# zlib-ng/minizip-ng

Measured on NVIDIA H100. Metric: deflate_l1_crc32_input_throughput, higher is better.
Workload: dtype u8

## Files before the change

### minizip-ng_b200/csrc/deflate_kernel.cuh

```cuda
#ifndef MZ_DEFLATE_KERNEL_CUH
#define MZ_DEFLATE_KERNEL_CUH

#include "mzcuda_common.cuh"

namespace mzc {

constexpr int DF_THREADS = 512;
constexpr int DF_WARPS = DF_THREADS / 32;
constexpr int DF_CHUNK_MAX = 65536;
constexpr int DF_UNIT = 32768;
constexpr int DF_SB = DF_UNIT;
constexpr int DF_SPAN = 8;
constexpr int DF_BATCH = DF_THREADS * DF_SPAN;
constexpr int DF_NBATCH = DF_UNIT / DF_BATCH;
constexpr int DF_MINMATCH = 4;
constexpr int DF_LOCKLEN = 8;
constexpr int DF_HASH_BITS = 13;
constexpr int DF_HASH_ENTRIES = 1 << DF_HASH_BITS;
constexpr int DF_STAGE_WORDS = DF_UNIT / 4 + 64;
constexpr int DF_HDR_WORDS = 96;

constexpr uint32_t DF_FLAG_FINAL = 1u;
constexpr uint32_t DF_FLAG_DICT = 2u;

constexpr int DF_OFF_IN = 0;
constexpr int DF_OFF_HASH = DF_OFF_IN + DF_UNIT + 64;
constexpr int DF_OFF_STAGE = DF_OFF_HASH;
constexpr int DF_OFF_REC = DF_OFF_HASH + DF_STAGE_WORDS * 4;
constexpr int DF_OFF_SPN = DF_OFF_REC + DF_NBATCH * DF_THREADS * 8;
constexpr int DF_SPAN_BYTES = DF_NBATCH * DF_THREADS * 10;
constexpr int DF_OFF_HIST = DF_OFF_REC + DF_SPAN_BYTES;
constexpr int DF_OFF_HIST2 = DF_OFF_HIST + (288 + 32) * 4;
constexpr int DF_OFF_CODE = DF_OFF_HIST2 + 256 * 4;
constexpr int DF_OFF_LENS = DF_OFF_CODE + (288 + 32) * 4;
constexpr int DF_OFF_BITS = DF_OFF_LENS + (288 + 32);
constexpr int DF_OFF_SCAN = DF_OFF_BITS + (288 + 32);
constexpr int DF_OFF_BB = DF_OFF_SCAN + 256 * 4;
constexpr int DF_OFF_MISC = DF_OFF_BB + 512 * 4;
constexpr int DF_OFF_SINK = DF_OFF_MISC + 32 * 4 + 16;
constexpr int DF_OFF_LSYM = DF_OFF_SINK + 32 * 4;
constexpr int DF_SMEM_BYTES = DF_OFF_LSYM + 256 * 2;
constexpr int DF_OFF_CAPL = DF_OFF_HIST;
static_assert(DF_OFF_CAPL + DF_WARPS * DF_NBATCH * 32 <= DF_OFF_SCAN, "capped-span lists fit in front of the scan scratch");
constexpr uint32_t DF_ZERO_SYM = 286;
static_assert(DF_HASH_ENTRIES * 4 <= DF_STAGE_WORDS * 4, "hash fits the staging region");
constexpr int DFH_PREV = 32768;
constexpr int DFH_HASH_BITS = 14;
constexpr int DFH_OFF_HASH = (DF_SMEM_BYTES + 15) & ~15;
constexpr int DFH_SMEM_BYTES = DFH_PREV + DFH_OFF_HASH + (4 << DFH_HASH_BITS);
static_assert(DFH_SMEM_BYTES <= 227 * 1024, "shared memory budget of the history variant");
static_assert(DF_SMEM_BYTES <= 113 * 1024, "shared memory budget for two CTAs per SM");

enum { MISC_CHUNK = 3, MISC_CARRY = 8  };

struct DeflateParams {
    const uint8_t *in;
    const uint64_t *in_off;
    const uint32_t *in_len;
    const uint8_t *flags;
    uint64_t total_len;
    uint32_t chunk_size;
    uint32_t nchunks;
    uint32_t last_flags;
    int32_t level;
    uint8_t *out;
    uint64_t slot_stride;
    uint32_t *out_len;
    uint32_t *work_counter;
};

__host__ __device__ inline uint64_t deflate_slot_bound(uint32_t chunk_size) {
    return (((uint64_t)chunk_size + 12ull * ((chunk_size + DF_SB - 1) / DF_SB + 1) + 64 + 15) & ~15ull);
}

__device__ __forceinline__ void length_symbol(uint32_t len, uint32_t &sym, uint32_t &ebits, uint32_t &eval) {
    const uint32_t l = len - 3;
    const uint32_t msb = 31u - (uint32_t)__clz((int)(l | 4u));
    uint32_t e = msb - 2;
    uint32_t sy = 4 * (e + 1) + ((l >> e) & 3u);
    uint32_t ev = l & ((1u << e) - 1u);
    sy = l < 8 ? l : sy;
    const bool top = len == 258;
    sym = top ? 28u : sy;
    ebits = top ? 0u : e;
    eval = top ? 0u : ev;
}
__device__ __forceinline__ void dist_symbol0(uint32_t d, uint32_t &sym, uint32_t &ebits) {
    uint32_t m = 31u - (uint32_t)__clz((int)(d | 1u));
    ebits = m > 0 ? m - 1 : 0u;
    sym = 2 * m + ((d >> ebits) & 1u);
}
__device__ __forceinline__ uint32_t len_extra_bits(uint32_t lsym) { return (lsym < 8 || lsym >= 28) ? 0u : (lsym >> 2) - 1; }
__device__ __forceinline__ uint32_t dist_extra_bits(uint32_t dsym) { return dsym < 4 ? 0u : (dsym >> 1) - 1; }

__device__ __forceinline__ uint32_t stage_word(uint32_t base, uint32_t pos, uint32_t k4) { return base + __umulhi(pos, 1u << 27) * k4; }

__device__ __forceinline__ void stage_put(uint32_t *stage, uint32_t pos, uint32_t v, uint32_t n) {
    if (n == 0) return;
    if (n < 32) v &= (1u << n) - 1;
    uint32_t w = pos >> 5, s = pos & 31;
    atomicOr(&stage[w], v << s);
    if (s + n > 32) atomicOr(&stage[w + 1], v >> (32 - s));
}

__device__ __forceinline__ void stage_or(const Smem &sm, uint32_t pos, uint32_t v, uint32_t n) {
    const uint32_t sh = pos & 31u, wa = DF_OFF_STAGE + ((pos >> 5) << 2);
    sm.red_or32(wa, v << sh);
    if (sh + n > 32) sm.red_or32(wa + 4, v >> (32 - sh));
}

struct BitWriter {
    Smem sm;
    uint64_t acc;
    uint32_t nb, wa;
    __device__ __forceinline__ void init(const Smem &s, uint32_t bitoff) {
        sm = s; wa = DF_OFF_STAGE + (bitoff >> 5) * 4; nb = bitoff & 31; acc = 0;
    }
    __device__ __forceinline__ void put(uint32_t v, uint32_t n) {
        acc |= (uint64_t)v << nb;
        nb += n;
        if (nb >= 32) {
            sm.red_or32(wa, (uint32_t)acc);
            acc >>= 32; nb -= 32; wa += 4;
        }
    }
    __device__ __forceinline__ uint32_t bitpos() const { return ((wa - (uint32_t)DF_OFF_STAGE) << 3) + nb; }
    __device__ __forceinline__ void finish() {
        if (nb > 0) sm.red_or32(wa, (uint32_t)acc);
        if (nb > 32) sm.red_or32(wa + 4, (uint32_t)(acc >> 32));
    }
};

enum { DF_PH_LOAD, DF_PH_PARSE, DF_PH_M0, DF_PH_COVER, DF_PH_T_M1, DF_PH_D, DF_PH_EMIT, DF_PH_FLUSH, DF_PH_UNITS,
       DF_PH_D_STATS, DF_PH_D_SWEEP1, DF_PH_D_SWEEP2, DF_PH_D_KRAFT, DF_PH_D_CANON, DF_PH_D_PASSES,
       DF_PH_P_A = DF_PH_D_PASSES + 8, DF_PH_P_B, DF_PH_P_C, DF_PH_M_INDEX, DF_PH_M_NEAR, DF_PH_M_EXTEND, DF_PH_X_SCAN, DF_PH_X_EMIT,
       DF_PH_X_M3, DF_PH_COLS };
constexpr int DF_PH_ROWS = 1024;
#if defined(MZ_DF_PHASES) && !defined(MZ_EMU)
__device__ unsigned long long g_df_phases[DF_PH_ROWS][DF_PH_COLS];
#define DF_PHASE_BEGIN(t) unsigned long long t = clock64()
#define DF_PHASE(t, ph)                                                                        \
    do {                                                                                       \
        if (threadIdx.x == 0 && blockIdx.x < (unsigned)DF_PH_ROWS) {                           \
            const unsigned long long now_ = clock64();                                         \
            atomicAdd(&g_df_phases[blockIdx.x][ph], now_ - (t));                               \
            if ((ph) == DF_PH_LOAD) atomicAdd(&g_df_phases[blockIdx.x][DF_PH_UNITS], 1ull);   \
            (t) = now_;                                                                        \
        }                                                                                      \
    } while (0)
#define DF_PHASE_COUNT(col)                                                                                          \
    do {                                                                                                             \
        if (threadIdx.x == 0 && blockIdx.x < (unsigned)DF_PH_ROWS) atomicAdd(&g_df_phases[blockIdx.x][col], 1ull); \
    } while (0)
#else
#define DF_PHASE_BEGIN(t)
#define DF_PHASE(t, ph)
#define DF_PHASE_COUNT(col)
#endif

constexpr int DF_BB_THREADS = 320;
enum { BB_STAT = 0 , BB_KRAFT = 8 , BB_SLACK = 136 ,
       BB_CNTW = 144 ,
       BB_NZ = 464 , BB_ST = 474 ,
       BB_HSUM = 484 , BB_HDRBITS = 494 ,
       BB_TOKBITS = 495 , BB_TOKW = 496  };

constexpr uint64_t CL_LENS = 0x12ddad91b725bb4ull;
constexpr uint64_t CL_CODE_LO = 0x840013930ef3c6ull, CL_CODE_HI = 0xd5c7fdf6cb149ull;
constexpr uint64_t CL_ORDER57 = 0x1b6d6db248db92dull;
__device__ __forceinline__ uint32_t cl_len(uint32_t s) { return (uint32_t)(CL_LENS >> (3 * s)) & 7u; }
__device__ __forceinline__ uint32_t cl_code(uint32_t s) {
    return s < 10 ? (uint32_t)(CL_CODE_LO >> (6 * s)) & 63u : (uint32_t)(CL_CODE_HI >> (6 * (s - 10))) & 63u;
}

__device__ __forceinline__ void bb_count_lengths(uint32_t *cntw_row, uint32_t L, unsigned lane, unsigned &m) {
    if (lane < 16) cntw_row[lane] = 0;
    __syncwarp();
    m = __match_any_sync(MZ_FULL_MASK, L);
    if (L > 0 && lane == (unsigned)(__ffs((int)m) - 1)) cntw_row[L] = (uint32_t)__popc(m);
    __syncwarp();
}

__device__ inline void block_build_codes(const uint32_t *hist_ll, const uint32_t *hist_lit2, const uint32_t *hist_d, uint8_t *lens_ll, uint8_t *lens_d,
                                         uint32_t *code_ll, uint32_t *code_d, uint8_t *bits_ll, uint8_t *bits_d, uint32_t *bb,
                                         uint32_t *stage, uint32_t hdrpos, uint32_t bfinal) {
    const uint32_t tid = threadIdx.x;
    const unsigned lane = lane_id(), w = warp_id();
    const int a = tid < 288 ? 0 : (tid < 320 ? 1 : 2);
    const uint32_t sym = a == 0 ? tid : tid - 288;
    const uint32_t nsym = a == 0 ? 286u : 30u;
    const int M = 15;
    const uint32_t one = 1u << M;
    const uint32_t w0 = a == 0 ? 0u : 9u;
    uint32_t c = (a < 2 && sym < nsym) ? (a == 0 ? hist_ll[sym] + (sym < 256 ? hist_lit2[sym] : 0u) : hist_d[sym]) : 0u;
    DF_PHASE_BEGIN(d_t);

    if (tid < 144) bb[tid] = (tid == BB_STAT + 2 || tid == BB_STAT + 6) ? 0xffffffffu : 0u;
    bar_sync(1, DF_BB_THREADS);
    if (a < 2) {
        uint32_t used_w = __reduce_add_sync(MZ_FULL_MASK, c ? 1u : 0u);
        uint32_t tot_w = __reduce_add_sync(MZ_FULL_MASK, c);
        uint32_t first_w = __reduce_min_sync(MZ_FULL_MASK, c ? sym : 0xffffffffu);
        if (lane == 0) {
            atomicAdd(&bb[BB_STAT + a * 4 + 0], used_w);
            atomicAdd(&bb[BB_STAT + a * 4 + 1], tot_w);
            atomicMin(&bb[BB_STAT + a * 4 + 2], first_w);
        }
    }
    bar_sync(1, DF_BB_THREADS);
    DF_PHASE(d_t, DF_PH_D_STATS);
    float ideal = 0.f;
    if (a < 2) {
        uint32_t used = bb[BB_STAT + a * 4 + 0], total = bb[BB_STAT + a * 4 + 1], fu = bb[BB_STAT + a * 4 + 2];
        if (used < 2) {
            uint32_t d0 = used == 0 ? 0u : (fu == 0 ? 1u : 0u);
            uint32_t d1 = used == 0 ? 1u : d0;
            if ((sym == d0 || sym == d1) && c == 0) c = 1;
            total += 2 - used;
        }
// ... 217 lines not shown
        len += 4;
    }
    return len < maxlen ? len : maxlen;
}

__device__ __forceinline__ uint32_t sel_u32(bool p, uint32_t a, uint32_t b) {
#ifdef MZ_EMU
    return p ? a : b;
#else
    uint32_t r;
    asm("{\n.reg .pred q;\nsetp.ne.u32 q, %3, 0;\nselp.b32 %0, %1, %2, q;\n}" : "=r"(r) : "r"(a), "r"(b), "r"((uint32_t)p));
    return r;
#endif
}

__device__ __forceinline__ uint32_t opaque4() { return blockDim.x / (uint32_t)(DF_THREADS / 4); }

template <bool HIST>
__device__ __forceinline__ uint32_t hash_addr(uint32_t v, uint32_t k4) {
    return (HIST ? DFH_OFF_HASH : DF_OFF_HASH) + __umulhi(v * 2654435761u, 1u << (HIST ? DFH_HASH_BITS : DF_HASH_BITS)) * k4;
}

__device__ __forceinline__ uint32_t rec_len(uint32_t r) { uint32_t l = (r >> 3) & 255u; return l ? l + 3 : 0u; }

__device__ __forceinline__ uint32_t fin_len(uint32_t m) { return ((m >> 4) & 255u) + 3u; }
__device__ __forceinline__ uint32_t fin_dist(uint32_t m) { return ((m >> 12) & 0x7fffu) + 1u; }
template <bool ONEM>
__device__ __forceinline__ void span_classify(const Smem &sm, uint32_t A, uint32_t B, uint32_t q0, uint32_t cover, uint32_t &F, uint32_t &MA,
                                              uint32_t &MB) {
    const uint32_t lit = (A >> 26) | ((B >> 26) << 6);
    const uint32_t crel = cover > q0 ? cover - q0 : 0u;
    const uint32_t cr8 = crel < 8 ? crel : 8u;
    uint32_t ex = 0;
    MA = MB = 0;
#pragma unroll
    for (int r = 0; r < (ONEM ? 1 : 2); r++) {
        const uint32_t R = r == 0 ? A : B;
        const uint32_t j = R & 7u, end = j + rec_len(R);
        const uint32_t s = j > crel ? j : crel;
        const uint32_t Lf = (end > s ? end : s) - s;
        const uint32_t P = (s < 8u ? s : 8u) & 7u;
        const uint32_t M = Lf >= 3 ? (((Lf << 4) + (0x80000000u - (3u << 4))) | P | ((R << 1) & (0x7fffu << 12))) : 0u;
        if (r == 0) MA = M;
        else MB = M;
        ex = Lf - 1u < 2u ? Lf : ex;
    }
    F = ((lit >> cr8) << cr8) | (ex << 8);
    if (ex) {
        const uint32_t p = DF_OFF_IN + q0 + crel;
        F |= sm.ld8(p) << 16;
        if (ex == 2) F |= sm.ld8(p + 1) << 24;
    }
}

__device__ __forceinline__ uint32_t match_symbols(const Smem &sm, uint32_t M) {
    uint32_t ds, db;
    const uint32_t lsv = sm.ld16(DF_OFF_LSYM + ((M >> 3) & 0x1feu));
    const uint32_t d = fin_dist(M) - 1;
    dist_symbol0(d, ds, db);
    sm.red_add32(DF_OFF_HIST + (257u + (lsv & 31u)) * 4, 1u);
    sm.red_add32(DF_OFF_HIST + (288u + ds) * 4, 1u);
    return 0x80000000u | ((M & 7u) << 28) | ((d & ((1u << db) - 1u)) << 15) | (ds << 10) | lsv;
}
__device__ __forceinline__ uint32_t match_bits(const Smem &sm, uint32_t M) {
    const uint32_t n = sm.ld8(DF_OFF_BITS + 257u + (M & 31u)) + sm.ld8(DF_OFF_BITS + 288u + ((M >> 10) & 31u));
    return M ? n : 0u;
}
__device__ __forceinline__ void put_match_bits(const Smem &sm, uint32_t pos, uint32_t M) {
    const uint32_t cwl = sm.ld32(DF_OFF_CODE + (257u + (M & 31u)) * 4);
    const uint32_t cwd = sm.ld32(DF_OFF_CODE + (288u + ((M >> 10) & 31u)) * 4);
    const uint32_t cl = (cwl >> 16) & 15u, cd = (cwd >> 16) & 15u;
    const uint32_t v1 = (cwl & 0x7fffu) | (((M >> 5) & 31u) << cl);
    const uint32_t n1 = cl + ((cwl >> 20) & 15u);
    const uint32_t v2 = (cwd & 0x7fffu) | (((M >> 15) & 0x1fffu) << cd);
    const uint64_t V = (uint64_t)v1 | ((uint64_t)v2 << n1);
    const uint32_t lo = (uint32_t)V, hi = (uint32_t)(V >> 32);
    const uint32_t wa = stage_word(DF_OFF_STAGE, pos, opaque4());
    const uint32_t w0 = __funnelshift_l(0u, lo, pos), w1 = __funnelshift_l(lo, hi, pos), w2 = __funnelshift_l(hi, 0u, pos);
    sm.red_or32(wa, w0);
    sm.red_or32(wa + 4, w1);
    if (w2) sm.red_or32(wa + 8, w2);
}

__device__ __forceinline__ uint32_t nth_parked(const uint32_t (&bm)[DF_NBATCH], uint32_t k, uint32_t warp) {
    uint32_t r = k, word = 0, bsel = 0;
    bool found = false;
#pragma unroll
    for (int b = 0; b < DF_NBATCH; b++) {
        const uint32_t c = (uint32_t)__popc(bm[b]);
        const bool here = !found && r < c;
        word = here ? bm[b] : word;
        bsel = here ? (uint32_t)b : bsel;
        found = found || here;
        r -= found ? 0u : c;
    }
    uint32_t base = 0;
#pragma unroll
    for (int st = 16; st; st >>= 1) {
        const uint32_t c = (uint32_t)__popc((word >> base) & ((1u << st) - 1u));
        const bool up = r >= c;
        r -= up ? c : 0u;
        base += up ? (uint32_t)st : 0u;
    }
    return found ? bsel * (uint32_t)DF_THREADS + warp * 32u + base : 0xffffffffu;
}

struct SpanBits {
    uint32_t v[4], E0, E1, offs, xv, MA, size;
};
template <bool ONEM>
__device__ __forceinline__ SpanBits span_bits(const Smem &sm, uint32_t sidx, uint32_t F, uint32_t MA, uint32_t MB, uint32_t code_base, uint32_t zero_ent,
                                              uint32_t k4) {
    SpanBits s;
    const uint2 x = sm.ld64(DF_OFF_IN + sidx * DF_SPAN);
    uint32_t xn = 0;
    s.xv = 0;
    const uint32_t ex = (F >> 8) & 3u;
    if (ex) {
        const uint32_t c0 = sm.ld32(DF_OFF_CODE + ((F >> 16) & 0xffu) * 4);
        s.xv = c0 & 0x7fffu;
        xn = (c0 >> 16) & 15u;
        if (ex == 2) {
            const uint32_t c1 = sm.ld32(DF_OFF_CODE + (F >> 24) * 4);
            s.xv |= (c1 & 0x7fffu) << xn;
            xn += (c1 >> 16) & 15u;
        }
    }
    uint32_t cw[8];
#pragma unroll
    for (int j = 0; j < 8; j++) {
        const uint32_t by = MZ_BYTE(j < 4 ? x.x : x.y, j & 3);
        cw[j] = sm.ld32_a(((F >> j) & 1u) ? by * k4 + code_base : zero_ent);
    }
    const uint32_t nA = match_bits(sm, MA), nB = ONEM ? 0u : match_bits(sm, MB);
    const uint32_t sA = MA ? ((MA >> 28) & 7u) * 8u : 64u, sB = MB ? ((MB >> 28) & 7u) * 8u : 64u;
    const uint32_t L0 = __byte_perm(__byte_perm(cw[0], cw[1], 0x0062u), __byte_perm(cw[2], cw[3], 0x0062u), 0x5410u) + shl_clamp(nA, sA) + shl_clamp(nB, sB);
    const uint32_t L1 = __byte_perm(__byte_perm(cw[4], cw[5], 0x0062u), __byte_perm(cw[6], cw[7], 0x0062u), 0x5410u) + shl_clamp(nA, sA - 32u) + shl_clamp(nB, sB - 32u);
    const uint32_t P0 = L0 * 0x01010101u;
    const uint32_t P1 = L1 * 0x01010101u + (P0 >> 24) * 0x01010101u;
    s.E0 = P0 << 8;
    s.E1 = __funnelshift_l(P0, P1, 8);
#pragma unroll
    for (int jj = 0; jj < 4; jj++) {
        const uint32_t c0 = cw[2 * jj], c1 = cw[2 * jj + 1];
        s.v[jj] = (c0 & 0xffffu) | ((c1 & 0xffffu) << (c0 >> 16));
    }
    s.offs = xn + (((shr_clamp(s.E0, sA) & 0xffu) + (shr_clamp(s.E1, sA - 32u) & 0xffu)) << 8) +
             (((shr_clamp(s.E0, sB) & 0xffu) + (shr_clamp(s.E1, sB - 32u) & 0xffu)) << 16);
    s.MA = MA;
    s.size = xn + (P1 >> 24);
    return s;
}
template <bool ONEM>
__device__ __forceinline__ void span_emit(const Smem &sm, const SpanBits &s, uint32_t pos, uint32_t sidx, uint32_t stage_base, uint32_t k4) {
    const uint32_t xn = s.offs & 0xffu;
    if (xn) stage_or(sm, pos, s.xv, xn);
    pos += xn;
#pragma unroll
    for (int jj = 0; jj < 4; jj++) {
        const uint32_t pp = pos + MZ_BYTE(jj < 2 ? s.E0 : s.E1, 2 * (jj & 1));
        const uint32_t wa = stage_word(stage_base, pp, k4);
        sm.red_or32_a(wa, __funnelshift_l(0u, s.v[jj], pp));
        sm.red_or32_a(wa + 4, __funnelshift_l(s.v[jj], 0u, pp));
    }
    if (s.MA) put_match_bits(sm, pos + ((s.offs >> 8) & 0xffu), s.MA);
    if (!ONEM) sm.st32(DF_OFF_REC + sidx * 8, pos + (s.offs >> 16));
}

template <int STRIDE, bool LAZY, bool HIST = false>
__global__ void __launch_bounds__(DF_THREADS, HIST ? 1 : 2) deflate_chunks_kernel(DeflateParams P) {
    MZ_DYN_SMEM(smem_raw);
    uint8_t *const smem = smem_raw + (HIST ? DFH_PREV : 0);
    constexpr uint32_t CUR = HIST ? (uint32_t)DFH_PREV : 0u;
    uint8_t *s_in = smem + DF_OFF_IN;
    uint32_t *s_stage = (uint32_t *)(smem + DF_OFF_STAGE);
    uint32_t *s_hist_ll = (uint32_t *)(smem + DF_OFF_HIST);
    uint32_t *s_hist_d = s_hist_ll + 288;
    uint32_t *s_code_ll = (uint32_t *)(smem + DF_OFF_CODE);
    uint32_t *s_code_d = s_code_ll + 288;
    uint8_t *s_lens_ll = smem + DF_OFF_LENS;
    uint8_t *s_lens_d = s_lens_ll + 288;
    uint8_t *s_bits_ll = smem + DF_OFF_BITS;
    uint8_t *s_bits_d = s_bits_ll + 288;
    uint32_t *s_scan = (uint32_t *)(smem + DF_OFF_SCAN);
    uint32_t *s_bb = (uint32_t *)(smem + DF_OFF_BB);
    uint32_t *s_misc = (uint32_t *)(smem + DF_OFF_MISC);
#ifndef MZ_EMU
    uint64_t *s_bar = (uint64_t *)(smem + DF_OFF_MISC + 32 * 4);
    uint32_t bar_phase = 0;
    if (threadIdx.x == 0) {
        mbar_init(s_bar, 1);
        mbar_fence_init();
    }
    __syncthreads();
#endif
    const uint32_t tid = threadIdx.x;
    const unsigned lane = lane_id(), warp = warp_id();
    Smem sm;
    sm.init(smem);
    if (tid < 256) {
        uint32_t ls, lb, lv;
        length_symbol(tid + 3, ls, lb, lv);
        sm.st16(DF_OFF_LSYM + tid * 2, ls | (lv << 5));
    }
    constexpr bool ONEM = false;
    DF_PHASE_BEGIN(ph_t);

    for (uint32_t chunk_static = blockIdx.x;; chunk_static += gridDim.x) {
        uint32_t chunk = chunk_static;
        if (P.work_counter) {
            if (tid == 0) s_misc[MISC_CHUNK] = atomicAdd(P.work_counter, 1u);
            __syncthreads();
            chunk = s_misc[MISC_CHUNK];
        }
        if (chunk >= P.nchunks) {
            if (P.work_counter && tid == 0 && atomicAdd(P.work_counter + 1, 1u) == gridDim.x - 1) {
                P.work_counter[0] = 0;
                P.work_counter[1] = 0;
            }
            break;
        }
        uint64_t off;
        uint32_t len, flags;
        if (P.in_off) {
            off = P.in_off[chunk];
            len = P.in_len[chunk];
            flags = P.flags ? P.flags[chunk] : 0u;
        } else {
            off = (uint64_t)chunk * P.chunk_size;
            uint64_t rem = P.total_len - off;
            len = rem < P.chunk_size ? (uint32_t)rem : P.chunk_size;
            flags = P.flags ? P.flags[chunk] : ((chunk == P.nchunks - 1 ? P.last_flags & ~DF_FLAG_DICT : 0u) | (P.last_flags & DF_FLAG_DICT));
        }
        const bool dict = HIST && (flags & DF_FLAG_DICT) && off >= (uint64_t)DFH_PREV;
        uint8_t *gout = P.out + (uint64_t)chunk * P.slot_stride;

        uint32_t flushed = 0;
        uint32_t bitpos = 0;
        const uint32_t nunits = (len + DF_UNIT - 1) / DF_UNIT;
        if (tid < 4) s_misc[MISC_CARRY + tid] = 0;

        if (len == 0) {
            for (uint32_t i = tid; i < 64; i += DF_THREADS) s_stage[i] = 0;
            __syncthreads();
            if (flags & DF_FLAG_FINAL) {
                if (tid == 0) stage_put(s_stage, 0, 1u | (1u << 1), 3);
                bitpos = 10;
            }
            __syncthreads();
        }

        for (uint32_t u = 0; u < nunits; u++) {
            const uint32_t ustart = u * DF_UNIT;
            const uint32_t ulen = (ustart + DF_UNIT < len) ? (uint32_t)DF_UNIT : len - ustart;
            const uint8_t *gin = P.in + off + ustart;
            const bool last_unit = u == nunits - 1;
            const uint32_t nb = (ulen + DF_BATCH - 1) / DF_BATCH;

            const uint32_t len16 = ulen & ~15u;
            bool bulk = false;
#ifndef MZ_EMU
            bulk = (((uintptr_t)gin) & 15) == 0 && len16 > 0;
            if (bulk && tid == 0) {
                fence_proxy_async();
                mbar_expect_tx(s_bar, len16);
                tma_load_1d(s_in, gin, len16, s_bar);
            }
#endif
            if (!bulk) {
                if ((((uintptr_t)gin) & 15) == 0) {
                    for (uint32_t i = tid * 16; i < len16; i += DF_THREADS * 16) *(uint4 *)(s_in + i) = ldg_stream((const uint4 *)(gin + i));
                } else {
                    for (uint32_t i = tid; i < len16; i += DF_THREADS) s_in[i] = gin[i];
                }
            }
            for (uint32_t i = len16 + tid; i < ulen; i += DF_THREADS) s_in[i] = gin[i];
            for (uint32_t i = ulen + tid; i < ((ulen + 63) & ~15u) + 16 && i < DF_UNIT + 64; i += DF_THREADS) s_in[i] = 0;
            if (P.level != 0) {
                if (!HIST) {
                    for (uint32_t i = tid; i < DF_HASH_ENTRIES / 4; i += DF_THREADS) sm.st128(DF_OFF_HASH + i * 16, ~0u, ~0u, ~0u, ~0u);
                } else if (u == 0) {
                    for (uint32_t i = tid; i < (1u << DFH_HASH_BITS) / 4; i += DF_THREADS) sm.st128(DFH_OFF_HASH + i * 16, ~0u, ~0u, ~0u, ~0u);
                    if (dict) {
                        const uint8_t *gp = P.in + off - DFH_PREV;
                        if ((((uintptr_t)gp) & 15) == 0) {
                            for (uint32_t i = tid * 16; i < (uint32_t)DFH_PREV; i += DF_THREADS * 16) *(uint4 *)(smem - DFH_PREV + i) = ldg_stream((const uint4 *)(gp + i));
                        } else {
                            for (uint32_t i = tid; i < (uint32_t)DFH_PREV; i += DF_THREADS) smem[(int)i - DFH_PREV] = gp[i];
                        }
                    }
                } else {
                    for (uint32_t i = tid; i < (1u << DFH_HASH_BITS) / 4; i += DF_THREADS) {
                        uint4 e = *(const uint4 *)(smem + DFH_OFF_HASH + i * 16);
                        e.x = (e.x != ~0u && (e.x & 0xffffu) >= (uint32_t)DFH_PREV) ? e.x + 0x78000u : ~0u;
                        e.y = (e.y != ~0u && (e.y & 0xffffu) >= (uint32_t)DFH_PREV) ? e.y + 0x78000u : ~0u;
                        e.z = (e.z != ~0u && (e.z & 0xffffu) >= (uint32_t)DFH_PREV) ? e.z + 0x78000u : ~0u;
                        e.w = (e.w != ~0u && (e.w & 0xffffu) >= (uint32_t)DFH_PREV) ? e.w + 0x78000u : ~0u;
                        *(uint4 *)(smem + DFH_OFF_HASH + i * 16) = e;
                    }
                }
            }
#ifndef MZ_EMU
            if (bulk) {
                mbar_wait(s_bar, bar_phase);
                bar_phase ^= 1;
            }
#endif
            __syncthreads();
            if (HIST && P.level != 0 && u == 0 && dict) {
#pragma unroll 1
                for (uint32_t b = 0; b < (uint32_t)DF_NBATCH; b++) {
                    const uint32_t p0 = b * DF_BATCH + tid * DF_SPAN;
                    const uint2 x = sm.ld64((uint32_t)(DF_OFF_IN - DFH_PREV) + p0);
                    const uint32_t y = sm.ld32((uint32_t)(DF_OFF_IN - DFH_PREV) + p0 + 8);
                    const uint32_t key0 = ((15u - b) << 16) | p0;
#pragma unroll
                    for (int j = 0; j < 8; j++) {
                        const uint32_t v = j == 0 ? x.x : (j < 4 ? __funnelshift_r(x.x, x.y, 8 * j) : (j == 4 ? x.y : __funnelshift_r(x.y, y, 8 * (j - 4))));
                        sm.red_min32(hash_addr<true>(v, 4u), key0 + j);
                    }
                }
                __syncthreads();
            }
            DF_PHASE(ph_t, DF_PH_LOAD);

            uint32_t fF[DF_NBATCH], fA[DF_NBATCH];
            bool stored = (P.level == 0);
            const uint32_t bfinal = (last_unit && (flags & DF_FLAG_FINAL)) ? 1u : 0u;

            if (P.level != 0) {
                DF_PHASE_BEGIN(p_t);
                uint32_t ncap = 0;
#pragma unroll 1
                for (uint32_t b = 0; b < nb; b++) {
                    const uint32_t q0 = b * DF_BATCH + tid * DF_SPAN;
                    uint32_t v[12], ha[8], lc[8];
                    const uint32_t k4 = opaque4();
                    {
                        const uint2 x = sm.ld64(DF_OFF_IN + q0), y = sm.ld64(DF_OFF_IN + q0 + 8);
                        v[0] = x.x; v[4] = x.y; v[8] = y.x;
#pragma unroll
                        for (int k = 1; k < 4; k++) {
                            v[k] = __funnelshift_r(x.x, x.y, 8 * k);
                            v[4 + k] = __funnelshift_r(x.y, y.x, 8 * k);
                            v[8 + k] = __funnelshift_r(y.x, y.y, 8 * k);
                        }
                    }
#pragma unroll
                    for (int j = 0; j < 8; j++) {
                        ha[j] = hash_addr<HIST>(v[j], k4);
                        if (j % STRIDE == 0) lc[j] = sm.ld32(ha[j]);
                    }
                    const uint32_t nvalid = ulen > q0 ? (ulen - q0 < 8 ? ulen - q0 : 8u) : 0u;
                    __syncthreads();
                    DF_PHASE(p_t, DF_PH_P_A);
                    const uint32_t key0 = ((uint32_t)(DF_NBATCH - 1 - b) << 16) | (CUR + q0);
#pragma unroll
                    for (int j = 0; j < 8; j++) sm.red_min32(ha[j], key0 + j);
                    __syncthreads();
                    DF_PHASE(p_t, DF_PH_P_B);
#pragma unroll
                    for (int j = 0; j < 8; j++) {
                        if (j % STRIDE != 0) {
                            lc[j] = 0;
                            continue;
                        }
                        const uint32_t kp = key0 + j, kn = sm.ld32(ha[j]);
                        const uint32_t ck = kn < kp ? kn : lc[j];
                        const uint32_t c = HIST ? ck & 0xffffu : ck;
                        const uint32_t ca = DF_OFF_IN - CUR + (c & 0xfffcu);
                        const uint32_t w0 = sm.ld32(ca), w1 = sm.ld32(ca + 4), w2 = sm.ld32(ca + 8);
                        const uint32_t s = c << 3;
                        const uint32_t x0 = __funnelshift_r(w0, w1, s) ^ v[j];
                        const uint32_t x1 = __funnelshift_r(w1, w2, s) ^ v[j + 4];
                        const bool reach = HIST ? c < CUR + q0 + j && c >= q0 + j : ck != 0xffffffffu;
                        const uint32_t l3 = ((uint32_t)__clz((int)__brev(x1)) & ~7u) + 8u;
                        lc[j] = sel_u32(reach && x0 == 0, (((kp - ck - 1u) << 11) & (0x7fffu << 11)) + l3 + (uint32_t)j, 0u);
                    }
                    if (q0 + 16 > ulen) {
#pragma unroll
                        for (int j = 0; j < 8; j += STRIDE) {
                            const uint32_t room = ulen > q0 + j ? ulen - (q0 + j) : 0u;
                            const uint32_t l = rec_len(lc[j]);
                            lc[j] = l >= (uint32_t)DF_MINMATCH && l > room ? (room >= (uint32_t)DF_MINMATCH ? lc[j] - ((l - room) << 3) : 0u) : lc[j];
                        }
                    }
                    uint32_t nxt = 0, lit = 0, mA = 0, mB = 0, span_end = 0;
                    if (STRIDE == 2 && !LAZY && !ONEM) {
#pragma unroll
                        for (int j = 6; j >= 0; j -= 2) mA = lc[j] ? lc[j] : mA;
                        const uint32_t endA = (mA & 7u) + rec_len(mA);
#pragma unroll
                        for (int j = 6; j >= 2; j -= 2) mB = lc[j] && (uint32_t)j >= endA ? lc[j] : mB;
                        const uint32_t endB = (mB & 7u) + rec_len(mB);
                        lit = ~(((1u << endA) - (1u << (mA & 7u))) | ((1u << endB) - (1u << (mB & 7u)))) & 0xffu;
                        span_end = mB ? endB : endA;
                    } else {
#pragma unroll
                        for (int j = 0; j < 8; j++) {
                            const bool take = nxt == (uint32_t)j;
                            if (j % STRIDE == 0) {
                                const uint32_t rec = lc[j], l = rec_len(rec);
                                bool ism = take && rec != 0;
                                if (LAZY && STRIDE == 1 && j < 7) ism = ism && !(((lc[j + 1] >> 3) & 255u) > ((rec >> 3) & 255u));
                                const bool first = mA == 0;
                                if (ONEM) ism = ism && first;
                                mA = (ism && first) ? rec : mA;
                                if (!ONEM) mB = (ism && !first) ? rec : mB;
                                lit |= (take && !ism) ? (1u << j) : 0u;
// ... 57 lines not shown
                                            sm.st64(DF_OFF_REC + sidx * 8, mA | ((lit & 63u) << 26), (lit >> 6) << 26);
                                            sm.st16(DF_OFF_SPN + sidx * 2, mA ? ((mA & 7u) << 9) | ((mA & 7u) + rec_len(mA)) : 0u);
                                            continue;
                                        }
                                        l = extend_match8(sm, cn, q, maxlen);
                                        cb = cn;
                                    }
                                }
                            }
                            DF_PHASE(m_t, DF_PH_M_NEAR);
                            if (l < 64u && l < maxlen) {
                                const uint32_t lf = extend_match8(sm, c, q, maxlen);
                                if (lf > l) {
                                    l = lf;
                                    cb = c;
                                }
                            }
                            sm.st32(DF_OFF_REC + sidx * 8 + (second ? 4u : 0u), (w & ~((255u << 3) | (0x7fffu << 11))) | ((l - 3) << 3) | ((q - cb - 1u) << 11));
                            sm.st16(DF_OFF_SPN + sidx * 2, (j << 9) | (j + l));
                            DF_PHASE(m_t, DF_PH_M_EXTEND);
                        }
                    }
                }
                __syncthreads();
                DF_PHASE(ph_t, DF_PH_M0);

                for (uint32_t i = tid; i < DF_STAGE_WORDS / 4; i += DF_THREADS) {
                    if (i == 0) sm.st128(DF_OFF_STAGE, s_misc[MISC_CARRY], s_misc[MISC_CARRY + 1], s_misc[MISC_CARRY + 2], s_misc[MISC_CARRY + 3]);
                    else sm.st128(DF_OFF_STAGE + i * 16, 0, 0, 0, 0);
                }
                for (uint32_t i = tid; i < 288 + 32 + 256; i += DF_THREADS) s_hist_ll[i] = 0;

                {
                    uint32_t se[8];
                    if (tid * 8 < nb * DF_THREADS) {
                        const uint4 q = *(const uint4 *)(smem + DF_OFF_SPN + tid * 16);
                        se[0] = q.x & 0xffffu; se[1] = q.x >> 16; se[2] = q.y & 0xffffu; se[3] = q.y >> 16;
                        se[4] = q.z & 0xffffu; se[5] = q.z >> 16; se[6] = q.w & 0xffffu; se[7] = q.w >> 16;
                    } else {
#pragma unroll
                        for (int k = 0; k < 8; k++) se[k] = 0;
                    }
                    const uint32_t p0 = tid * 64;
                    uint32_t tmax = 0;
#pragma unroll
                    for (int k = 0; k < 8; k++) {
                        const uint32_t e = se[k] ? p0 + 8 * k + (se[k] & 511u) : 0u;
                        tmax = tmax > e ? tmax : e;
                    }
                    const uint32_t incl = warp_incl_max(tmax);
                    uint32_t cin = __shfl_up_sync(MZ_FULL_MASK, incl, 1);
                    if (lane == 0) cin = 0;
                    if (lane == 31) s_scan[warp] = incl;
                    __syncthreads();
                    {
                        const uint32_t w = (lane < (unsigned)DF_WARPS && lane < warp) ? s_scan[lane] : 0u;
                        const uint32_t base = __reduce_max_sync(MZ_FULL_MASK, w);
                        cin = cin > base ? cin : base;
                    }
                    uint32_t run = cin, drop = 0, pcv = 0, pendk = 0;
                    bool alive = false;
                    uint32_t cv[8];
#pragma unroll
                    for (int k = 0; k < 8; k++) {
                        const uint32_t q0 = p0 + 8 * k;
                        const uint32_t ms = q0 + (se[k] >> 9), me = q0 + (se[k] & 511u);
                        const bool fc = run >= q0 + 8;
                        const bool strad = se[k] != 0 && ms < run && me > run;
                        const bool takes = fc && strad && alive && ms <= pcv;
                        drop |= takes ? 1u << pendk : 0u;
                        cv[k] = takes ? pcv : run;
                        pcv = (fc && strad && !takes) ? run : pcv;
                        pendk = (fc && strad) ? (uint32_t)k : pendk;
                        alive = fc && (strad || alive);
                        run = (se[k] != 0 && me > run) ? me : run;
                    }
#pragma unroll
                    for (int k = 0; k < 8; k++) cv[k] = ((drop >> k) & 1u) ? 0xffffu : cv[k];
                    *(uint4 *)(smem + DF_OFF_SPN + tid * 16) = make_uint4(cv[0] | (cv[1] << 16), cv[2] | (cv[3] << 16), cv[4] | (cv[5] << 16), cv[6] | (cv[7] << 16));
                }
                __syncthreads();
                DF_PHASE(ph_t, DF_PH_COVER);

                const uint32_t hist_lit = sm.addr((lane & 1u) ? (uint32_t)DF_OFF_HIST2 : (uint32_t)DF_OFF_HIST);
                const uint32_t k4 = opaque4();
                const uint32_t sink = sm.addr(DF_OFF_SINK + lane * 4);
                uint32_t bmB[DF_NBATCH];
#pragma unroll
                for (int b = 0; b < DF_NBATCH; b++) {
                    uint32_t F = 0, MA = 0, MB = 0;
                    bmB[b] = 0;
                    if ((uint32_t)b < nb) {
                        const uint32_t sidx = (uint32_t)b * DF_THREADS + tid;
                        const uint32_t q0 = sidx * DF_SPAN;
                        const uint2 r = sm.ld64(DF_OFF_REC + sidx * 8);
                        const uint32_t cover = sm.ld16(DF_OFF_SPN + sidx * 2);
                        span_classify<ONEM>(sm, r.x, r.y, q0, cover, F, MA, MB);
                        const uint32_t ex = (F >> 8) & 3u;
                        if (ex) {
                            sm.red_add32_a(hist_lit + ((F >> 16) & 0xffu) * 4, 1u);
                            if (ex == 2) sm.red_add32_a(hist_lit + (F >> 24) * 4, 1u);
                        }
                        const uint2 x = sm.ld64(DF_OFF_IN + q0);
#pragma unroll
                        for (int j = 0; j < 8; j++) {
                            const uint32_t by = MZ_BYTE(j < 4 ? x.x : x.y, j & 3);
                            sm.red_add32_a(((F >> j) & 1u) ? by * k4 + hist_lit : sink, 1u);
                        }
                        if (MA) MA = match_symbols(sm, MA);
                        if (!ONEM) {
                            bmB[b] = __ballot_sync(MZ_FULL_MASK, MB != 0);
                            sm.st32(DF_OFF_REC + sidx * 8 + 4, MB);
                        }
                    }
                    fF[b] = F; fA[b] = MA;
                }
                if (!ONEM) {
                    uint32_t totB = 0;
#pragma unroll
                    for (int b = 0; b < DF_NBATCH; b++) totB += (uint32_t)__popc(bmB[b]);
                    __syncwarp();
                    for (uint32_t k0 = 0; k0 < totB; k0 += 32) {
                        const uint32_t sidx = nth_parked(bmB, k0 + lane, warp);
                        if (sidx != 0xffffffffu) {
                            const uint32_t a = DF_OFF_REC + sidx * 8 + 4;
                            sm.st32(a, match_symbols(sm, sm.ld32(a)));
                        }
                    }
                }
                if (tid == 0) sm.red_add32(DF_OFF_HIST + 256 * 4, 1u);
                __syncthreads();
                DF_PHASE(ph_t, DF_PH_T_M1);
#ifdef MZ_DF_CODES_HOOK
                if (tid == 0) MZ_DF_CODES_HOOK(s_hist_ll, (const uint32_t *)(smem + DF_OFF_HIST2), s_hist_d);
#endif
                if (tid < DF_BB_THREADS)
                    block_build_codes(s_hist_ll, (const uint32_t *)(smem + DF_OFF_HIST2), s_hist_d, s_lens_ll, s_lens_d, s_code_ll, s_code_d, s_bits_ll, s_bits_d, s_bb,
                                      s_stage, bitpos, bfinal);
                __syncthreads();
                DF_PHASE(ph_t, DF_PH_D);
                const uint32_t hdrbits = s_bb[BB_HDRBITS], tokbits = s_bb[BB_TOKBITS];
                const uint32_t eob = s_code_ll[256];
                const uint32_t dyn_bits = hdrbits + tokbits + ((eob >> 16) & 15u);
                const uint32_t stored_bits = (((bitpos + 3 + 7) & ~7u) - bitpos) + 32 + ulen * 8;
                if (dyn_bits >= stored_bits) {
                    stored = true;
                    const uint32_t w0 = bitpos >> 5;
                    for (uint32_t i = tid; i <= (hdrbits + 31) / 32 + 1; i += DF_THREADS)
                        s_stage[w0 + i] = i == 0 ? s_stage[w0] & ((1u << (bitpos & 31u)) - 1u) : 0u;
                    __syncthreads();
                } else {
                    const uint32_t code_base = sm.addr(DF_OFF_CODE), zero_ent = sm.addr(DF_OFF_CODE + DF_ZERO_SYM * 4), stage_base = sm.addr(DF_OFF_STAGE);
                    const uint32_t k4 = opaque4();
                    uint32_t run = bitpos + hdrbits;
                    DF_PHASE_BEGIN(x_t);
#pragma unroll
                    for (int b = 0; b < DF_NBATCH; b += 2) {
                        if ((uint32_t)b >= nb) break;
                        const uint32_t s0 = (uint32_t)b * DF_THREADS + tid, s1 = s0 + DF_THREADS;
                        const uint32_t MB0 = ONEM ? 0u : sm.ld32(DF_OFF_REC + s0 * 8 + 4);
                        const uint32_t MB1 = (ONEM || (uint32_t)b + 1 >= nb) ? 0u : sm.ld32(DF_OFF_REC + s1 * 8 + 4);
                        const SpanBits A = span_bits<ONEM>(sm, s0, fF[b], fA[b], MB0, code_base, zero_ent, k4);
                        const SpanBits B = span_bits<ONEM>(sm, s1, fF[b + 1], fA[b + 1], MB1, code_base, zero_ent, k4);
                        const uint32_t sz = A.size | (B.size << 16);
                        const uint32_t incl = warp_incl_sum(sz);
                        if (lane == 31) s_scan[(b / 2) * DF_WARPS + warp] = incl;
                        __syncthreads();
                        DF_PHASE(x_t, DF_PH_X_SCAN);
                        const uint32_t wt = lane < (unsigned)DF_WARPS ? s_scan[(b / 2) * DF_WARPS + lane] : 0u;
                        const uint32_t wlo = wt & 0xffffu, whi = wt >> 16;
                        const uint32_t totA = __reduce_add_sync(MZ_FULL_MASK, wlo);
                        const uint32_t ex = incl - sz;
                        const uint32_t posA = run + __reduce_add_sync(MZ_FULL_MASK, lane < warp ? wlo : 0u) + (ex & 0xffffu);
                        const uint32_t posB = run + totA + __reduce_add_sync(MZ_FULL_MASK, lane < warp ? whi : 0u) + (ex >> 16);
                        run += totA + __reduce_add_sync(MZ_FULL_MASK, whi);
                        if (A.size) span_emit<ONEM>(sm, A, posA, s0, stage_base, k4);
                        if (B.size) span_emit<ONEM>(sm, B, posB, s1, stage_base, k4);
                        DF_PHASE(x_t, DF_PH_X_EMIT);
                    }
#ifdef MZ_EMU
                    if (run != bitpos + hdrbits + tokbits) {
                        fprintf(stderr, "deflate: block %u, unit %u: emitted %u token bits, the histograms count %u\n", (unsigned)blockIdx.x, u,
                                run - bitpos - hdrbits, tokbits);
                        abort();
                    }
#endif
                    if (!ONEM) {
                        uint32_t totB = 0;
#pragma unroll
                        for (int b = 0; b < DF_NBATCH; b++) totB += (uint32_t)__popc(bmB[b]);
                        __syncwarp();
                        for (uint32_t k0 = 0; k0 < totB; k0 += 32) {
                            const uint32_t sidx = nth_parked(bmB, k0 + lane, warp);
                            if (sidx != 0xffffffffu) {
                                const uint2 r = sm.ld64(DF_OFF_REC + sidx * 8);
                                put_match_bits(sm, r.x, r.y);
                            }
                        }
                    }
                    DF_PHASE(x_t, DF_PH_X_M3);
                    if (tid == DF_THREADS - 1) stage_put(s_stage, bitpos + hdrbits + tokbits, eob & 0x7fffu, (eob >> 16) & 15u);
                    bitpos += dyn_bits;
                }
            } else {
                for (uint32_t i = tid; i < DF_STAGE_WORDS / 4; i += DF_THREADS) {
                    if (i == 0) sm.st128(DF_OFF_STAGE, s_misc[MISC_CARRY], s_misc[MISC_CARRY + 1], s_misc[MISC_CARRY + 2], s_misc[MISC_CARRY + 3]);
                    else sm.st128(DF_OFF_STAGE + i * 16, 0, 0, 0, 0);
                }
                __syncthreads();
            }
            if (stored) {
                const uint32_t p0 = (bitpos + 3 + 7) >> 3;
                if (tid == 0) {
                    stage_put(s_stage, bitpos, bfinal, 3);
                    stage_put(s_stage, p0 * 8, ulen, 16);
                    stage_put(s_stage, p0 * 8 + 16, ulen ^ 0xffffu, 16);
                }
                for (uint32_t i = tid * 4; i < ulen; i += DF_THREADS * 4) {
                    uint32_t v = load32u(s_in, i);
                    uint32_t n = ulen - i;
                    stage_put(s_stage, (p0 + 4 + i) * 8, v, n >= 4 ? 32 : n * 8);
                }
                bitpos = (p0 + 4 + ulen) * 8;
            }
            __syncthreads();
            DF_PHASE(ph_t, DF_PH_EMIT);
            {
                const uint32_t n16 = bitpos >> 7;
                const uint32_t used_words = (bitpos + 31) >> 5;
#pragma unroll 4
                for (uint32_t i = tid; i < n16; i += DF_THREADS) ((uint4 *)(gout + flushed))[i] = ((const uint4 *)s_stage)[i];
                if (tid < 4) s_misc[MISC_CARRY + tid] = (n16 * 4 + tid < used_words) ? s_stage[n16 * 4 + tid] : 0u;
                bitpos -= n16 * 128;
                flushed += n16 * 16;
                if (HIST && u + 1 < nunits)
                    for (uint32_t i = tid; i < (uint32_t)DF_UNIT / 16; i += DF_THREADS) *(uint4 *)(smem - DFH_PREV + i * 16) = *(const uint4 *)(s_in + i * 16);
                __syncthreads();
                DF_PHASE(ph_t, DF_PH_FLUSH);
            }
        }


        {
            if (tid < 8) {
                const uint32_t v = tid < 4 ? (len == 0 ? s_stage[tid] : s_misc[MISC_CARRY + tid]) : 0u;
                __syncwarp(0xffu);
                s_stage[tid] = v;
            }
            __syncthreads();
            if (flags & DF_FLAG_FINAL) {
                bitpos = (bitpos + 7) & ~7u;
            } else {
                const uint32_t p0 = (bitpos + 3 + 7) >> 3;
                if (tid == 0) stage_put(s_stage, (p0 + 2) * 8, 0xffffu, 16);
                bitpos = (p0 + 4) * 8;
            }
            __syncthreads();
            if (tid < 8) ((uint32_t *)(gout + flushed))[tid] = s_stage[tid];
            if (tid == 0) P.out_len[chunk] = flushed + (bitpos >> 3);
            __syncthreads();
            DF_PHASE(ph_t, DF_PH_FLUSH);
        }
    }
}

__host__ __device__ inline int deflate_stride_for_level(int level) { return level <= 1 ? 2 : 1; }
__host__ __device__ inline bool deflate_lazy_for_level(int level) { return level >= 4; }
__host__ __device__ inline bool deflate_hist_for_level(int level) { return level >= 6; }

}
#endif
```

Measured before the change: 161.8.

## Defer all match symbol coding to compacted per-warp lists instead of per-span lanes

After: 164.6, median of 6. 1.02x the previous value.

```diff
diff --git a/minizip-ng_b200/csrc/deflate_kernel.cuh b/minizip-ng_b200/csrc/deflate_kernel.cuh
--- a/minizip-ng_b200/csrc/deflate_kernel.cuh
+++ b/minizip-ng_b200/csrc/deflate_kernel.cuh
@@ -42,6 +42,11 @@
 constexpr int DF_SMEM_BYTES = DF_OFF_LSYM + 256 * 2;
 constexpr int DF_OFF_CAPL = DF_OFF_HIST;
 static_assert(DF_OFF_CAPL + DF_WARPS * DF_NBATCH * 32 <= DF_OFF_SCAN, "capped-span lists fit in front of the scan scratch");
+static_assert(DF_OFF_HIST - DF_OFF_SPN == DF_NBATCH * DF_THREADS * 2, "a warp's covers of a batch are 64 bytes: two lists of 32 entries");
+__device__ __forceinline__ uint32_t match_list(uint32_t warp, uint32_t k) {
+    return DF_OFF_SPN + warp * 64u + k + (k >> 5) * (uint32_t)(DF_THREADS * 2 - 32);
+}
+constexpr uint32_t DF_LIST_B = 32;
 constexpr uint32_t DF_ZERO_SYM = 286;
 static_assert(DF_HASH_ENTRIES * 4 <= DF_STAGE_WORDS * 4, "hash fits the staging region");
 constexpr int DFH_PREV = 32768;
@@ -50,6 +55,8 @@
 constexpr int DFH_SMEM_BYTES = DFH_PREV + DFH_OFF_HASH + (4 << DFH_HASH_BITS);
 static_assert(DFH_SMEM_BYTES <= 227 * 1024, "shared memory budget of the history variant");
 static_assert(DF_SMEM_BYTES <= 113 * 1024, "shared memory budget for two CTAs per SM");
+template <bool HIST>
+__device__ __forceinline__ uint32_t park_base() { return HIST ? (uint32_t)(DF_OFF_IN - DFH_PREV) : (uint32_t)DF_OFF_IN; }
 
 enum { MISC_CHUNK = 3, MISC_CARRY = 8  };
 
@@ -131,10 +138,10 @@
     }
 };
 
-enum { DF_PH_LOAD, DF_PH_PARSE, DF_PH_M0, DF_PH_COVER, DF_PH_T_M1, DF_PH_D, DF_PH_EMIT, DF_PH_FLUSH, DF_PH_UNITS,
+enum { DF_PH_LOAD, DF_PH_PARSE, DF_PH_M0, DF_PH_COVER, DF_PH_T, DF_PH_D, DF_PH_EMIT, DF_PH_FLUSH, DF_PH_UNITS,
        DF_PH_D_STATS, DF_PH_D_SWEEP1, DF_PH_D_SWEEP2, DF_PH_D_KRAFT, DF_PH_D_CANON, DF_PH_D_PASSES,
        DF_PH_P_A = DF_PH_D_PASSES + 8, DF_PH_P_B, DF_PH_P_C, DF_PH_M_INDEX, DF_PH_M_NEAR, DF_PH_M_EXTEND, DF_PH_X_SCAN, DF_PH_X_EMIT,
-       DF_PH_X_M3, DF_PH_COLS };
+       DF_PH_X_M3, DF_PH_T_CLASS, DF_PH_T_MATCH, DF_PH_COLS };
 constexpr int DF_PH_ROWS = 1024;
 #if defined(MZ_DF_PHASES) && !defined(MZ_EMU)
 __device__ unsigned long long g_df_phases[DF_PH_ROWS][DF_PH_COLS];
@@ -518,31 +525,14 @@
     if (w2) sm.red_or32(wa + 8, w2);
 }
 
-__device__ __forceinline__ uint32_t nth_parked(const uint32_t (&bm)[DF_NBATCH], uint32_t k, uint32_t warp) {
-    uint32_t r = k, word = 0, bsel = 0;
-    bool found = false;
-#pragma unroll
-    for (int b = 0; b < DF_NBATCH; b++) {
-        const uint32_t c = (uint32_t)__popc(bm[b]);
-        const bool here = !found && r < c;
-        word = here ? bm[b] : word;
-        bsel = here ? (uint32_t)b : bsel;
-        found = found || here;
-        r -= found ? 0u : c;
-    }
-    uint32_t base = 0;
-#pragma unroll
-    for (int st = 16; st; st >>= 1) {
-        const uint32_t c = (uint32_t)__popc((word >> base) & ((1u << st) - 1u));
-        const bool up = r >= c;
-        r -= up ? c : 0u;
-        base += up ? (uint32_t)st : 0u;
-    }
-    return found ? bsel * (uint32_t)DF_THREADS + warp * 32u + base : 0xffffffffu;
+__device__ __forceinline__ uint32_t match_word(const Smem &sm, uint32_t warp, uint32_t k, uint32_t nA) {
+    const bool second = k >= nA;
+    const uint32_t e = sm.ld8(match_list(warp, second ? k - nA : k) + (second ? DF_LIST_B : 0u));
+    return e * 8u + (e >> 5) * (uint32_t)(DF_THREADS * 8 - 256) + warp * 256u + (second ? 4u : 0u);
 }
 
 struct SpanBits {
-    uint32_t v[4], E0, E1, offs, xv, MA, size;
+    uint32_t v[4], E0, E1, offs, xv, size;
 };
 template <bool ONEM>
 __device__ __forceinline__ SpanBits span_bits(const Smem &sm, uint32_t sidx, uint32_t F, uint32_t MA, uint32_t MB, uint32_t code_base, uint32_t zero_ent,
@@ -583,12 +573,10 @@
     }
     s.offs = xn + (((shr_clamp(s.E0, sA) & 0xffu) + (shr_clamp(s.E1, sA - 32u) & 0xffu)) << 8) +
              (((shr_clamp(s.E0, sB) & 0xffu) + (shr_clamp(s.E1, sB - 32u) & 0xffu)) << 16);
-    s.MA = MA;
     s.size = xn + (P1 >> 24);
     return s;
 }
-template <bool ONEM>
-__device__ __forceinline__ void span_emit(const Smem &sm, const SpanBits &s, uint32_t pos, uint32_t sidx, uint32_t stage_base, uint32_t k4) {
+__device__ __forceinline__ void span_emit(const Smem &sm, const SpanBits &s, uint32_t pos, uint32_t park, uint32_t stage_base, uint32_t k4) {
     const uint32_t xn = s.offs & 0xffu;
     if (xn) stage_or(sm, pos, s.xv, xn);
     pos += xn;
@@ -599,8 +587,7 @@
         sm.red_or32_a(wa, __funnelshift_l(0u, s.v[jj], pp));
         sm.red_or32_a(wa + 4, __funnelshift_l(s.v[jj], 0u, pp));
     }
-    if (s.MA) put_match_bits(sm, pos + ((s.offs >> 8) & 0xffu), s.MA);
-    if (!ONEM) sm.st32(DF_OFF_REC + sidx * 8, pos + (s.offs >> 16));
+    sm.st64(park, pos + ((s.offs >> 8) & 0xffu), pos + (s.offs >> 16));
 }
 
 template <int STRIDE, bool LAZY, bool HIST = false>
@@ -760,7 +747,7 @@
             }
             DF_PHASE(ph_t, DF_PH_LOAD);
 
-            uint32_t fF[DF_NBATCH], fA[DF_NBATCH];
+            uint32_t fF[DF_NBATCH];
             bool stored = (P.level == 0);
             const uint32_t bfinal = (last_unit && (flags & DF_FLAG_FINAL)) ? 1u : 0u;
 
@@ -984,14 +971,15 @@
                 __syncthreads();
                 DF_PHASE(ph_t, DF_PH_COVER);
 
+                DF_PHASE_BEGIN(t_t);
                 const uint32_t hist_lit = sm.addr((lane & 1u) ? (uint32_t)DF_OFF_HIST2 : (uint32_t)DF_OFF_HIST);
                 const uint32_t k4 = opaque4();
                 const uint32_t sink = sm.addr(DF_OFF_SINK + lane * 4);
-                uint32_t bmB[DF_NBATCH];
+                const uint32_t below = (1u << lane) - 1u;
+                uint32_t nA = 0, nB = 0;
 #pragma unroll
                 for (int b = 0; b < DF_NBATCH; b++) {
                     uint32_t F = 0, MA = 0, MB = 0;
-                    bmB[b] = 0;
                     if ((uint32_t)b < nb) {
                         const uint32_t sidx = (uint32_t)b * DF_THREADS + tid;
                         const uint32_t q0 = sidx * DF_SPAN;
@@ -1009,30 +997,29 @@
                             const uint32_t by = MZ_BYTE(j < 4 ? x.x : x.y, j & 3);
                             sm.red_add32_a(((F >> j) & 1u) ? by * k4 + hist_lit : sink, 1u);
                         }
-                        if (MA) MA = match_symbols(sm, MA);
-                        if (!ONEM) {
-                            bmB[b] = __ballot_sync(MZ_FULL_MASK, MB != 0);
-                            sm.st32(DF_OFF_REC + sidx * 8 + 4, MB);
-                        }
-                    }
-                    fF[b] = F; fA[b] = MA;
-                }
-                if (!ONEM) {
-                    uint32_t totB = 0;
-#pragma unroll
-                    for (int b = 0; b < DF_NBATCH; b++) totB += (uint32_t)__popc(bmB[b]);
-                    __syncwarp();
-                    for (uint32_t k0 = 0; k0 < totB; k0 += 32) {
-                        const uint32_t sidx = nth_parked(bmB, k0 + lane, warp);
-                        if (sidx != 0xffffffffu) {
-                            const uint32_t a = DF_OFF_REC + sidx * 8 + 4;
-                            sm.st32(a, match_symbols(sm, sm.ld32(a)));
-                        }
-                    }
-                }
+                        sm.st64(DF_OFF_REC + sidx * 8, MA, MB);
+                        const uint32_t bA = __ballot_sync(MZ_FULL_MASK, MA != 0), bB = __ballot_sync(MZ_FULL_MASK, MB != 0);
+                        __syncwarp();
+                        sm.st8_if(MA != 0, match_list(warp, nA + (uint32_t)__popc(bA & below)), ((uint32_t)b << 5) | lane);
+                        sm.st8_if(MB != 0, match_list(warp, nB + (uint32_t)__popc(bB & below)) + DF_LIST_B, ((uint32_t)b << 5) | lane);
+                        nA += (uint32_t)__popc(bA);
+                        nB += (uint32_t)__popc(bB);
+                    }
+                    fF[b] = F;
+                }
+                DF_PHASE(t_t, DF_PH_T_CLASS);
+                __syncwarp();
+                for (uint32_t k0 = 0; k0 < nA + nB; k0 += 32) {
+                    const uint32_t k = k0 + lane;
+                    if (k < nA + nB) {
+                        const uint32_t a = DF_OFF_REC + match_word(sm, warp, k, nA);
+                        sm.st32(a, match_symbols(sm, sm.ld32(a)));
+                    }
+                }
+                DF_PHASE(t_t, DF_PH_T_MATCH);
                 if (tid == 0) sm.red_add32(DF_OFF_HIST + 256 * 4, 1u);
                 __syncthreads();
-                DF_PHASE(ph_t, DF_PH_T_M1);
+                DF_PHASE(ph_t, DF_PH_T);
 #ifdef MZ_DF_CODES_HOOK
                 if (tid == 0) MZ_DF_CODES_HOOK(s_hist_ll, (const uint32_t *)(smem + DF_OFF_HIST2), s_hist_d);
 #endif
@@ -1060,10 +1047,10 @@
                     for (int b = 0; b < DF_NBATCH; b += 2) {
                         if ((uint32_t)b >= nb) break;
                         const uint32_t s0 = (uint32_t)b * DF_THREADS + tid, s1 = s0 + DF_THREADS;
-                        const uint32_t MB0 = ONEM ? 0u : sm.ld32(DF_OFF_REC + s0 * 8 + 4);
-                        const uint32_t MB1 = (ONEM || (uint32_t)b + 1 >= nb) ? 0u : sm.ld32(DF_OFF_REC + s1 * 8 + 4);
-                        const SpanBits A = span_bits<ONEM>(sm, s0, fF[b], fA[b], MB0, code_base, zero_ent, k4);
-                        const SpanBits B = span_bits<ONEM>(sm, s1, fF[b + 1], fA[b + 1], MB1, code_base, zero_ent, k4);
+                        const uint2 R0 = sm.ld64(DF_OFF_REC + s0 * 8), R1 = sm.ld64(DF_OFF_REC + s1 * 8);
+                        const bool none1 = (uint32_t)b + 1 >= nb;
+                        const SpanBits A = span_bits<ONEM>(sm, s0, fF[b], R0.x, R0.y, code_base, zero_ent, k4);
+                        const SpanBits B = span_bits<ONEM>(sm, s1, fF[b + 1], none1 ? 0u : R1.x, none1 ? 0u : R1.y, code_base, zero_ent, k4);
                         const uint32_t sz = A.size | (B.size << 16);
                         const uint32_t incl = warp_incl_sum(sz);
                         if (lane == 31) s_scan[(b / 2) * DF_WARPS + warp] = incl;
@@ -1076,8 +1063,8 @@
                         const uint32_t posA = run + __reduce_add_sync(MZ_FULL_MASK, lane < warp ? wlo : 0u) + (ex & 0xffffu);
                         const uint32_t posB = run + totA + __reduce_add_sync(MZ_FULL_MASK, lane < warp ? whi : 0u) + (ex >> 16);
                         run += totA + __reduce_add_sync(MZ_FULL_MASK, whi);
-                        if (A.size) span_emit<ONEM>(sm, A, posA, s0, stage_base, k4);
-                        if (B.size) span_emit<ONEM>(sm, B, posB, s1, stage_base, k4);
+                        if (A.size) span_emit(sm, A, posA, park_base<HIST>() + s0 * 8, stage_base, k4);
+                        if (B.size) span_emit(sm, B, posB, park_base<HIST>() + s1 * 8, stage_base, k4);
                         DF_PHASE(x_t, DF_PH_X_EMIT);
                     }
 #ifdef MZ_EMU
@@ -1087,17 +1074,12 @@
                         abort();
                     }
 #endif
-                    if (!ONEM) {
-                        uint32_t totB = 0;
-#pragma unroll
-                        for (int b = 0; b < DF_NBATCH; b++) totB += (uint32_t)__popc(bmB[b]);
-                        __syncwarp();
-                        for (uint32_t k0 = 0; k0 < totB; k0 += 32) {
-                            const uint32_t sidx = nth_parked(bmB, k0 + lane, warp);
-                            if (sidx != 0xffffffffu) {
-                                const uint2 r = sm.ld64(DF_OFF_REC + sidx * 8);
-                                put_match_bits(sm, r.x, r.y);
-                            }
+                    __syncwarp();
+                    for (uint32_t k0 = 0; k0 < nA + nB; k0 += 32) {
+                        const uint32_t k = k0 + lane;
+                        if (k < nA + nB) {
+                            const uint32_t w = match_word(sm, warp, k, nA);
+                            put_match_bits(sm, sm.ld32(park_base<HIST>() + w), sm.ld32(DF_OFF_REC + w));
                         }
                     }
                     DF_PHASE(x_t, DF_PH_X_M3);
```
